# biodatageeks/polars-bio

Measured on AMD Instinct MI355X. Metric: overlap-pairs/sec, higher is better.
Workload: dtype int32; 1 GPU; overlap_100M_5M_24contig; probe_rows=100000000, build_rows=5000000, contigs=24, filter_op=Strict, parallelism=single GPU

## Files before the change

polars-bio_amd/csrc/host_core.hip.h:

```cpp
#pragma once

namespace {

thread_local std::string g_err;

int fail(int code, const std::string& msg) { g_err = msg; return code; }

#define HIP_TRY(expr)                                                                         \
    do {                                                                                      \
        hipError_t _e = (expr);                                                               \
        if (_e != hipSuccess)                                                                 \
            return fail(IVJ_EHIP, std::string(#expr) + ": " + hipGetErrorString(_e));         \
    } while (0)

#define IVJ_ABI_CATCH                                                                                     \
    catch (const std::bad_alloc&) { return fail(IVJ_ENOMEM, "host allocation failed (std::bad_alloc)"); }   \
    catch (const std::exception& e) { return fail(IVJ_ESTATE, std::string("internal error: ") + e.what()); } \
    catch (...) { return fail(IVJ_ESTATE, "internal error: unknown exception"); }

#define IVJ_TRY(expr)                 \
    do {                              \
        int _r = (expr);              \
        if (_r != IVJ_OK) return _r;  \
    } while (0)
// ... 35 lines not shown
        }
    }
};

inline std::atomic<int> g_live_contexts{0};

struct ivj_ctx {
    ivj_ctx() { g_live_contexts.fetch_add(1, std::memory_order_relaxed); }
    ~ivj_ctx() { g_live_contexts.fetch_sub(1, std::memory_order_relaxed); }
    ivj_ctx(const ivj_ctx&) = delete;
    ivj_ctx& operator=(const ivj_ctx&) = delete;
    int device = 0;
    hipStream_t own_stream = nullptr;
    hipStream_t stream = nullptr;
    Arena arena;
    char* ov_buf = nullptr;
    size_t ov_cap = 0;
    int64_t ov_n = -1;
    const void* ov_probe_start = nullptr;
    const void *ov_probe_contig = nullptr, *ov_probe_end = nullptr;
    const ivj_index* ov_ix = nullptr;
    int32_t ov_filter = -1;
    int32_t* ov_hi = nullptr;
    int32_t* ov_cnt = nullptr;
    long long* ov_tile = nullptr;
    long long* h_total = nullptr;
    uint32_t* hw = nullptr;
    uint32_t* hw_dev = nullptr;
    uint32_t hw_seq = 0;
    uint32_t cs_far_hw_seq = 0;
    uint32_t cs_fused_hw_seq = 0;
    int env_spin_us = 4000;
    long long hw_misses = 0;
    bool cs_prep_zero = false;
    XferSlots xfer;
    char* nl_cache = nullptr;
    size_t nl_cache_cap = 0;
    int env_nearest_lines = -1;
    char* ix_cache = nullptr;
    size_t ix_cache_cap = 0;
    int64_t ov_total = 0;
    bool ov_part = false;
    int32_t *pt_c = nullptr, *pt_s = nullptr, *pt_e = nullptr, *pt_row = nullptr;
    uint32_t* pt_off = nullptr; int pt_ntiles = 0;
    uint32_t* pt_bstart = nullptr;
    bool part_attr_set = false;
    bool os_attr_set = false;
    hipEvent_t cs_event = nullptr;
    const ivj_index* cs_far_owner = nullptr;
    hipEvent_t ix3_event = nullptr;
    bool ix3_attr_set = false;
    int env_ix_merge = -1;
    int env_ix_stage = -1;
    int env_ix_v3 = -1;
    int ix3_fallback_streak = 0;
    unsigned ix3_builds_since_fallback = 0;
    int64_t ix3_fallbacks = 0;
    struct StreamBufs { int32_t* h_in = nullptr; int32_t* d_in = nullptr; size_t in_cap = 0; char* d_out = nullptr; size_t d_out_cap = 0;
                        char* h_out = nullptr; size_t h_out_cap = 0; } st_cache[3];
    char* lb_buf = nullptr; size_t lb_cap = 0;
    char* sel_buf = nullptr; size_t sel_cap = 0;
    char* sl_buf = nullptr;
    size_t sl_cap = 0;
    int4* sl_rec = nullptr;
    uint2* sl_cache = nullptr;
    uint32_t *sl_gh = nullptr, *sl_rstart = nullptr, *sl_rcur = nullptr, *sl_bend = nullptr;
    bool sl_sampled = false;
    uint32_t *sl_blk = nullptr, *sl_part = nullptr, *sl_bstart = nullptr;
    int32_t* sl_meta = nullptr;
    int2* sl_map = nullptr;
    long long *sl_tile = nullptr, *sl_tpart = nullptr;
    bool ov_slice = false;
    bool ov_cs = false;
    bool sl_plan_valid = false;
    int sl_items = 2;
    int env_joint_bins = 0, env_count_nolds = 0, env_count_ablate = 0;
    int sl_env_rows = 0, sl_env_chunk = 0, sl_env_notab = 0, sl_env_nobins = 0, sl_env_ablate = 0, sl_env_auto = 1, sl_env_stable = 0, sl_env_sthreads = 1024;
    SlicePlan sl_plan;
    bool cs_sattr_set = false;
    bool cs_attr_set = false;
    int cs_env_walk = -1;
    int cs_env_off = 0;
    int cs_env_ptile = 0;
    int cs_env_fill_two = 0;
    int cs_env_sampled = 1;
    int cs_env_slack = 0;
    int64_t cs_sampled_overflows = 0;
    bool cs_force_exact = false;
    int cs_env_fuse_sample = 1;
    int cs_env_rec8 = 1;
    bool cs_force_rec12 = false;
    int cs_rec8_streak = 0;
    unsigned cs_rec8_skipped = 0;
    bool cs_rec8_tried = false;
    int64_t cs_rec8_overflows = 0;
    int cs_env_nocache = 0;
    int cs_env_persist = 1;
    int cs_env_pmax = 0, cs_env_pgrain = 0;
    int cs_env_pchunks = 0;
    int n_cus = 0;
    const char* cs_env_wgtrace = nullptr;
    unsigned long long* cs_trace_buf = nullptr;
    size_t cs_trace_cap = 0;
    int timing = 0;
    bool t_open = false;
    std::vector<TimingRec> recs;
// ... 284 lines not shown
```

polars-bio_amd/csrc/host_index.hip.h:

```cpp
#pragma once

namespace {

int build_tables(ivj_ctx* ctx, ivj_index* ix);
bool cs_geom(int64_t n, int nc, int want_rows, CsGeom& g);
size_t cs_index_bytes(const CsGeom& g);
void cs_index_carve(ivj_index* ix, char* p);

int ensure_hier(ivj_ctx* ctx, ivj_index* ix) {
    if (ix->hier_built || ix->n <= 0) return IVJ_OK;
    const HierShape h = hier_shape(ix->n);
    const int64_t wgs = (((ix->n + 15) & ~(int64_t)15) + HIER_WG_ROWS - 1) / HIER_WG_ROWS;
    LAUNCH(ctx, "hier_low", k_hier_low, (unsigned)wgs, 256, (const int2*)ix->ep, ix->n, ix->hier, h);
    if (h.nlev >= 3) LAUNCH(ctx, "hier_high", k_hier_high, 1, 256, ix->hier, h, wgs);
    HIP_TRY(hipGetLastError());
    ix->hier_built = true;
    return IVJ_OK;
}

int need_tables(ivj_ctx* ctx, ivj_index* ix) {
    if (!ix->has_tables) return fail(IVJ_ESTATE, "this index was built for merge / cluster only (with_end_order & 2): it has no lookup tables");
    if (ix->tables_built) return IVJ_OK;
    return build_tables(ctx, ix);
}
// ... 176 lines not shown

int build_flat(ivj_ctx* ctx, ivj_index* ix) {
    if (ix->has_flat || ix->n == 0 || ix->n_contigs <= 0) return IVJ_OK;
    IVJ_TRY(need_tables(ctx, ix));
    HIP_TRY(hipMemsetAsync(ix->lot, 0, (size_t)ix->bins_len * 4, ctx->stream));
    LAUNCH(ctx, "lot_mark", k_lot_mark, grid1d(ix->n, 256), 256, (const int2*)ix->ep, (const int32_t*)ix->b_contig, ix->n,
           ix->n_contigs, (const int4*)ix->cmeta, ix->lot);
    IVJ_TRY((lb_scan_u32<MaxOp, false>(ctx, "lot_scan", ix->lot, ix->bins_len, 0u)));
    LAUNCH(ctx, "tab2", k_tab2, grid1d(ix->bins_len, 256), 256, (const uint32_t*)ix->bins, (const uint32_t*)ix->lot, ix->bins_len, ix->tab2);
    HIP_TRY(hipGetLastError());
    IVJ_TRY(build_rec4(ctx, ix));
    ix->has_flat = true;
    return IVJ_OK;
}

int index_sort_v2(ivj_ctx* ctx, ivj_index* ix, const ivj_side* build, const ivj_opts* opts) {
    OsSort S;
    IVJ_TRY(arena_reserve(ctx, os_sort_plan(S, build->n, opts->n_contigs) + 4096));
    os_sort_take(ctx, S);
    IVJ_TRY(os_sort_run(ctx, S, build->contig, build->start, build->end, build->row_id));
    LAUNCH(ctx, "ix_final", k_ix_final, S.tiles, OS_THREADS, (const int4*)S.recA, (const int4*)S.recB, S.n, S.nc, S.cbits, S.meta, S.st_fin, ix->b_start, ix->ep, ix->b_row,
           ix->b_contig, ix->seg, ix->flags);
    HIP_TRY(hipGetLastError());
    return IVJ_OK;
}

bool ix3_wanted(const ivj_ctx* ctx, int64_t n, int nc) {
    if (nc + 1 > V3_MAX_KEYS || n <= 0 || n > (int64_t)V3_CAP * V3_BUCKETS) return false;
    if (ctx->env_ix_v3 >= 0) return ctx->env_ix_v3 != 0;
    if (ctx->ix3_fallback_streak >= 2 && (ctx->ix3_builds_since_fallback & 15) != 15) return false;
    return n >= (128ll << 10) && n <= (7ll << 20);
}
struct V3Plan { int64_t chunk, hist_len, hs_tiles; int nchunks; size_t z_meta, z_st, z_hs, z_tick, zero_bytes; };
V3Plan v3_plan(int64_t n) {
    V3Plan p;
    p.chunk = ((n + 255) / 256 + OS_TILE - 1) / OS_TILE * OS_TILE;
    if (p.chunk < OS_TILE) p.chunk = OS_TILE;
    p.nchunks = (int)((n + p.chunk - 1) / p.chunk);
    p.hist_len = (int64_t)V3_BUCKETS * p.nchunks;
    p.hs_tiles = (p.hist_len + LB_TILE - 1) / LB_TILE;
    p.z_meta = align_up(sizeof(V3Meta)); p.z_st = align_up((size_t)V3_BUCKETS * 8); p.z_hs = align_up((size_t)p.hs_tiles * 8); p.z_tick = align_up(16);
    p.zero_bytes = p.z_meta + p.z_st + p.z_hs + p.z_tick;
    return p;
}
int index_sort_v3(ivj_ctx* ctx, ivj_index* ix, const ivj_side* build, const ivj_opts* opts, bool* done) {
    *done = false;
    const int64_t n = build->n;
    const int nc = opts->n_contigs;
    const int64_t tiles = (n + OS_TILE - 1) / OS_TILE;
    const V3Plan VP = v3_plan(n);
    const int64_t chunk = VP.chunk, hist_len = VP.hist_len, hs_tiles = VP.hs_tiles;
    const int nchunks = VP.nchunks;
    const size_t z_meta = VP.z_meta, z_st = VP.z_st, z_hs = VP.z_hs, zero_bytes = VP.zero_bytes;
    OsSort S;
    const size_t v2_bytes = os_sort_plan(S, n, nc);
    const bool own_z = ix->ix3_z == nullptr;
    IVJ_TRY(arena_reserve(ctx, std::max(v2_bytes, (own_z ? zero_bytes : 0) + align_up((size_t)hist_len * 4) + align_up((size_t)n * 16)) + 4096));
    char* z = own_z ? arena_take<char>(ctx, zero_bytes) : ix->ix3_z;
    uint32_t* hist = arena_take<uint32_t>(ctx, (size_t)hist_len);
    int4* recs = arena_take<int4>(ctx, (size_t)n);
    V3Meta* meta = (V3Meta*)z;
    unsigned long long* st_local = (unsigned long long*)(z + z_meta);
    unsigned long long* st_scan = (unsigned long long*)(z + z_meta + z_st);
    uint32_t* tick_scan = (uint32_t*)(z + z_meta + z_st + z_hs);
    if (own_z) HIP_TRY(hipMemsetAsync(z, 0, zero_bytes, ctx->stream));
    const size_t pass_lds = (size_t)v3_pass_lds().total;
    if (!ctx->ix3_attr_set) {
        HIP_TRY(hipFuncSetAttribute(reinterpret_cast<const void*>(&k_v3_scatter), hipFuncAttributeMaxDynamicSharedMemorySize, (int)pass_lds));
        HIP_TRY(hipFuncSetAttribute(reinterpret_cast<const void*>(&k_v3_local<true>), hipFuncAttributeMaxDynamicSharedMemorySize, 160 * 1024 - 256));
        HIP_TRY(hipFuncSetAttribute(reinterpret_cast<const void*>(&k_v3_local<false>), hipFuncAttributeMaxDynamicSharedMemorySize, 160 * 1024 - 256));
        ctx->ix3_attr_set = true;
    }
    const unsigned sgrid = (unsigned)(tiles < 512 ? tiles : 512);
    LAUNCH(ctx, "ix3_stats", k_v3_stats, sgrid, OS_THREADS, build->start, build->end, build->contig, n, nc, meta);
    LAUNCH(ctx, "ix3_hist", k_v3_hist, nchunks, OS_THREADS, build->contig, build->start, n, nc, meta, (int)chunk, nchunks, hist);
    LAUNCH(ctx, "ix_scan", (k_scan_lb_u32<SumOp, true>), hs_tiles, OS_THREADS, hist, hist_len, 0u, tick_scan, st_scan);
    const int ms_max = ctx->env_ix_merge >= 0 ? std::min(ctx->env_ix_merge, V3_MAX_MERGE) : V3_MAX_MERGE;
    const uint32_t hw_seq = ctx->hw ? ++ctx->hw_seq : 0u;
    LAUNCH(ctx, "ix3_check", k_v3_check, 1, OS_THREADS, (const uint32_t*)hist, nchunks, n, ms_max, meta, ctx->hw_dev, hw_seq);
    if (!ctx->hw) HIP_TRY(hipMemcpyAsync(ctx->h_total + 6, &meta->bad, 8, hipMemcpyDeviceToHost, ctx->stream));
    if (!ctx->ix3_event) HIP_TRY(hipEventCreateWithFlags(&ctx->ix3_event, hipEventDisableTiming));
    HIP_TRY(hipEventRecord(ctx->ix3_event, ctx->stream));
    t_begin(ctx, "ix3_pass");
    hipLaunchKernelGGL(k_v3_scatter, dim3((unsigned)nchunks), dim3(OS_THREADS), pass_lds, ctx->stream, build->contig, build->start, build->end, build->row_id,
                       recs, n, nc, meta, (int)chunk, nchunks, (const uint32_t*)hist);
    t_end(ctx);
    HIP_TRY(hipGetLastError());
    HIP_TRY(wait_event(ctx, ctx->ix3_event));
    uint32_t* hv = reinterpret_cast<uint32_t*>(ctx->h_total + 6);
    if (ctx->hw) {
        const volatile uint32_t* w = reinterpret_cast<volatile uint32_t*>(ctx->hw);
        if (w[2] == hw_seq) { hv[0] = w[0]; hv[1] = w[1]; }
        else {
            ++ctx->hw_misses;
            HIP_TRY(hipMemcpyAsync(ctx->h_total + 6, &meta->bad, 8, hipMemcpyDeviceToHost, ctx->stream));
            HIP_TRY(hipStreamSynchronize(ctx->stream));
        }
    }
    const uint32_t max_bucket = hv[1] & 0xffffffu;
    const int ms = (int)(hv[1] >> 24);
    if (hv[0] != 0u || max_bucket > (uint32_t)V3_CAP) { ++ctx->ix3_fallbacks; ++ctx->ix3_fallback_streak; ctx->ix3_builds_since_fallback = 0; return IVJ_OK; }
    ctx->ix3_fallback_streak = 0;
    const int cap = (int)std::max<uint32_t>(1024u, (max_bucket + 1023u) / 1024u * 1024u);
    const int bin_bits = cap <= 1024 ? 10 : (cap <= 2048 ? 11 : V3_MAX_BIN_BITS);
    const bool stage = ctx->env_ix_stage >= 0 ? ctx->env_ix_stage != 0 : cap <= 2048;
    const size_t local_lds = (size_t)v3_local_lds(cap, 1 << bin_bits, stage).total;
    with_bool(stage, [&](auto STAGE) {
        LAUNCH_LDS(ctx, "ix3_local", k_v3_local<STAGE>, V3_BUCKETS >> ms, OS_THREADS, local_lds, (const int4*)recs, (const uint32_t*)hist, nchunks, n, nc, cap, bin_bits, ms,
                   meta, st_local, ix->b_start, ix->ep, ix->b_row, ix->b_contig, ix->seg, ix->flags);
    });
    HIP_TRY(hipGetLastError());
    *done = true;
    return IVJ_OK;
}

int build_tables(ivj_ctx* ctx, ivj_index* ix) {
    const int nc = ix->n_contigs;
    const int64_t n = ix->n;
    if (n > 0 && nc > 0) {
        const int64_t lb_tiles = (ix->bins_len + LB_TILE - 1) / LB_TILE;
        const size_t zb = align_up((size_t)lb_tiles * 8) + align_up(16);
        IVJ_TRY(arena_reserve(ctx, zb + 4096));
        char* z = arena_take<char>(ctx, zb);
        HIP_TRY(hipMemsetAsync(z, 0, zb, ctx->stream));
        HIP_TRY(hipMemsetAsync(ix->bins, 0, (size_t)ix->bins_len * 4, ctx->stream));
        LAUNCH(ctx, "contig_meta", k_contig_meta, grid1d(nc, 256), 256, (const int32_t*)ix->seg, (const int32_t*)ix->b_start, nc, ix->cmeta);
        LAUNCH(ctx, "bins_mark", k_bins_mark, grid1d(n, 256), 256, (const int32_t*)ix->b_start, (const int32_t*)ix->b_contig, n, nc,
               (const int4*)ix->cmeta, ix->bins);
        LAUNCH(ctx, "bins_scan", (k_scan_lb_u32<MaxOp, false>), lb_tiles, OS_THREADS, ix->bins, ix->bins_len, 0u,
               (uint32_t*)(z + align_up((size_t)lb_tiles * 8)), (unsigned long long*)z);
        LAUNCH(ctx, "bins_records", k_bins_records, grid1d(ix->bins_len, 256), 256, (const uint32_t*)ix->bins, ix->bins_len,
               (const int32_t*)ix->b_start, (const int4*)ix->cmeta, nc, ix->brec);
        HIP_TRY(hipGetLastError());
    }
    ix->tables_built = true;
    return IVJ_OK;
}

int index_build(ivj_ctx* ctx, const ivj_side* build, const ivj_opts* opts, int with_end_order, ivj_index** out) {
    if (2 * build->n + 2 * (int64_t)opts->n_contigs + 64 > 0x7fffffffll)
        return fail(IVJ_EINVAL, "build side too large for the int32 direct-address table (2*rows + 2*contigs must be < 2^31)");
    ivj_index* ix = new ivj_index();
    ix->ctx = ctx; ix->device = ctx->device; ix->n = build->n; ix->n_contigs = opts->n_contigs; ix->table_mode = opts->table_mode;
    const int64_t n = build->n;
    const size_t nn = (size_t)(n > 0 ? n : 1);
    auto cleanup = [&](int code) { ivj_index_free(ix); return code; };
    {
        const size_t col = align_up(nn * 4);
        const size_t nc = (size_t)opts->n_contigs;
        ix->bins_len = 2 * (int64_t)nn + 2 * (int64_t)nc + 16;
        const size_t v3z = (n > 0 && ix3_wanted(ctx, n, opts->n_contigs)) ? v3_plan(n).zero_bytes : 0;
        const size_t small = align_up((nc + 2) * 4) + align_up(16) + 3 * align_up((nc + 1) * 32) + v3z;
        const size_t flat_bytes = align_up((nn + 1) * 16) + 3 * align_up((size_t)ix->bins_len * 4);
        const size_t spl_bytes = align_up((size_t)SL_MAX_BUCKETS * 8) + align_up((size_t)SL_TAB_CONTIGS * 16) +
                                 align_up((size_t)(4 * SL_MAX_BUCKETS + 2 * SL_TAB_CONTIGS) * 4);
        ix->cs_ok = n > 0 && cs_geom(n, opts->n_contigs, opts->slice_rows > 0 ? opts->slice_rows : ctx->sl_env_rows, ix->cs_g);
        const size_t cs_bytes = ix->cs_ok ? cs_index_bytes(ix->cs_g) : 0;
        const size_t hier_bytes = align_up(hier_shape((int64_t)nn).values * 4);
        const size_t need = hier_bytes + cs_bytes + spl_bytes + flat_bytes + 6 * col + align_up(nn * 8) + align_up((nn + 1) * 32) + 2 * align_up((size_t)ix->bins_len * 4) +
                            3 * align_up((size_t)ix->bins_len * 16) + small + 256;
        if (ctx->ix_cache && ctx->ix_cache_cap >= need) {
            ix->slab = ctx->ix_cache; ix->slab_cap = ctx->ix_cache_cap;
// ... 64 lines not shown
```

polars-bio_amd/csrc/ivjoin.hip:

```cpp
#include "../../include/ivjoin.h"

#include <hip/hip_runtime.h>

#include <algorithm>
#include <atomic>
#include <chrono>
#include <cstdio>
#include <cstdlib>
#include <cstring>
#include <string>
#include <vector>
#include <thread>
#include <type_traits>

#include "probe.hip.h"
#include "slice.hip.h"
#include "cslice.hip.h"
#include "onesweep.hip.h"
#include "ixsort3.hip.h"
#include "scan.hip.h"
#include "group.hip.h"
#include "depth.hip.h"
#include "depth_sum.hip.h"
#include "depth_query.hip.h"
// ... 34 lines not shown

int ivj_device_count(int* n) try {
    if (!n) return fail(IVJ_EINVAL, "n is NULL");
    int c = 0;
    hipError_t e = hipGetDeviceCount(&c);
    if (e != hipSuccess) { *n = 0; return fail(IVJ_EHIP, std::string("hipGetDeviceCount: ") + hipGetErrorString(e)); }
    *n = c;
    return IVJ_OK;
} IVJ_ABI_CATCH

int ivj_ctx_create(int device, ivj_ctx** out) try {
    if (!out) return fail(IVJ_EINVAL, "out is NULL");
    int cnt = 0;
    IVJ_TRY(ivj_device_count(&cnt));
    if (device < 0 || device >= cnt) return fail(IVJ_EHIP, "no usable HIP device " + std::to_string(device) + " (device count " + std::to_string(cnt) + ")");
    HIP_TRY(hipSetDevice(device));
    ivj_ctx* ctx = new ivj_ctx();
    ctx->device = device;
    { int cus = 0; if (hipDeviceGetAttribute(&cus, hipDeviceAttributeMultiprocessorCount, device) == hipSuccess) ctx->n_cus = cus; }
    hipError_t e = hipStreamCreateWithFlags(&ctx->own_stream, hipStreamNonBlocking);
    if (e != hipSuccess) { delete ctx; return fail(IVJ_EHIP, std::string("hipStreamCreate: ") + hipGetErrorString(e)); }
    ctx->stream = ctx->own_stream;
    if (const char* ev = std::getenv("IVJ_SLICE_ITEMS")) ctx->sl_items = std::atoi(ev) == 4 ? 4 : 2;
    if (const char* ev = std::getenv("IVJ_SLICE_ROWS")) ctx->sl_env_rows = std::atoi(ev);
    if (const char* ev = std::getenv("IVJ_SLICE_CHUNK")) ctx->sl_env_chunk = std::atoi(ev);
    if (const char* ev = std::getenv("IVJ_SLICE_NOTAB")) ctx->sl_env_notab = std::atoi(ev);
    if (const char* ev = std::getenv("IVJ_SLICE_NOBINS")) ctx->sl_env_nobins = std::atoi(ev);
    if (const char* ev = std::getenv("IVJ_SLICE_ABLATE")) ctx->sl_env_ablate = std::atoi(ev);
    if (const char* ev = std::getenv("IVJ_SLICE_AUTO")) ctx->sl_env_auto = std::atoi(ev);
    if (const char* ev = std::getenv("IVJ_SLICE_STABLE")) ctx->sl_env_stable = std::atoi(ev);
    if (const char* ev = std::getenv("IVJ_SLICE_SCATTER_THREADS")) ctx->sl_env_sthreads = std::atoi(ev);
    if (const char* ev = std::getenv("IVJ_CS")) ctx->cs_env_off = std::atoi(ev) == 0 ? 1 : 0;
    if (const char* ev = std::getenv("IVJ_CS_PTILE")) ctx->cs_env_ptile = std::atoi(ev);
    if (const char* ev = std::getenv("IVJ_CS_NOCACHE")) ctx->cs_env_nocache = std::atoi(ev);
    if (const char* ev = std::getenv("IVJ_CS_PERSIST")) ctx->cs_env_persist = std::atoi(ev);
    if (const char* ev = std::getenv("IVJ_CS_PCHUNKS")) ctx->cs_env_pchunks = std::atoi(ev);
    if (const char* ev = std::getenv("IVJ_CS_PMAX")) ctx->cs_env_pmax = std::atoi(ev);
    if (const char* ev = std::getenv("IVJ_CS_PGRAIN")) ctx->cs_env_pgrain = std::atoi(ev);
    if (const char* ev = std::getenv("IVJ_CS_WGTRACE")) ctx->cs_env_wgtrace = ev[0] ? ev : nullptr;
    if (const char* ev = std::getenv("IVJ_CS_SAMPLED")) ctx->cs_env_sampled = std::atoi(ev);
    if (const char* ev = std::getenv("IVJ_CS_SLACK")) ctx->cs_env_slack = std::atoi(ev);
    if (const char* ev = std::getenv("IVJ_CS_REC8")) ctx->cs_env_rec8 = std::atoi(ev);
    if (const char* ev = std::getenv("IVJ_CS_FUSE_SAMPLE")) ctx->cs_env_fuse_sample = std::atoi(ev);
    if (const char* ev = std::getenv("IVJ_CS_FILL_TWO")) ctx->cs_env_fill_two = std::atoi(ev);
    if (const char* ev = std::getenv("IVJ_CS_WALK")) ctx->cs_env_walk = std::atoi(ev) != 0 ? 1 : 0;
    if (const char* ev = std::getenv("IVJ_JOINT_BINS")) ctx->env_joint_bins = std::atoi(ev);
    if (const char* ev = std::getenv("IVJ_COUNT_ABLATE")) ctx->env_count_ablate = std::atoi(ev);
    if (const char* ev = std::getenv("IVJ_NEAREST_LINES")) ctx->env_nearest_lines = std::atoi(ev);
    if (const char* ev = std::getenv("IVJ_COUNT_NOLDS")) ctx->env_count_nolds = std::atoi(ev);
    if (const char* ev = std::getenv("IVJ_IX_V3")) ctx->env_ix_v3 = std::atoi(ev) != 0 ? 1 : 0;
    if (const char* ev = std::getenv("IVJ_SPIN_US")) ctx->env_spin_us = std::atoi(ev);
    if (const char* ev = std::getenv("IVJ_IX_MERGE")) ctx->env_ix_merge = std::atoi(ev);
    if (const char* ev = std::getenv("IVJ_IX_STAGE")) ctx->env_ix_stage = std::atoi(ev) != 0 ? 1 : 0;
    e = hipHostMalloc((void**)&ctx->h_total, 64, hipHostMallocDefault);
    if (e != hipSuccess) { (void)hipStreamDestroy(ctx->own_stream); delete ctx; return fail(IVJ_EHIP, std::string("hipHostMalloc: ") + hipGetErrorString(e)); }
    {
        const char* ev = std::getenv("IVJ_HOST_WORDS");
        if (!(ev && std::atoi(ev) == 0)) {
            void* hp = nullptr;
            void* dp = nullptr;
            if (hipHostMalloc(&hp, 256, hipHostMallocMapped | hipHostMallocCoherent) == hipSuccess) {
                if (hipHostGetDevicePointer(&dp, hp, 0) == hipSuccess && dp) {
                    std::memset(hp, 0, 256);
                    ctx->hw = (uint32_t*)hp; ctx->hw_dev = (uint32_t*)dp;
                } else (void)hipHostFree(hp);
            }
            (void)hipGetLastError();
        }
    }
    *out = ctx;
    return IVJ_OK;
} IVJ_ABI_CATCH

namespace {
void stream_release(ivj_stream* st, bool keep_cache);
void free_stream_bufs(ivj_ctx::StreamBufs& b) {
    if (b.h_in) (void)hipHostFree(b.h_in);
    if (b.d_in) (void)hipFree(b.d_in);
    if (b.d_out) (void)hipFree(b.d_out);
    if (b.h_out) (void)hipHostFree(b.h_out);
    b = ivj_ctx::StreamBufs();
}
}

void ivj_ctx_destroy(ivj_ctx* ctx) {
    if (!ctx) return;
    DeviceGuard g(ctx->device);
    (void)hipStreamSynchronize(ctx->stream);
    while (!ctx->streams.empty()) stream_release(ctx->streams.back(), false);
    for (ivj_index* ix : ctx->live) ix->ctx = nullptr;
    for (ivj_comm* cm : ctx->comms) comm_detach(cm);
    if (ctx->arena.base) (void)hipFree(ctx->arena.base);
    if (ctx->ov_buf) (void)hipFree(ctx->ov_buf);
    if (ctx->sl_buf) (void)hipFree(ctx->sl_buf);
    if (ctx->cs_trace_buf) (void)hipFree(ctx->cs_trace_buf);
    if (ctx->lb_buf) (void)hipFree(ctx->lb_buf);
    if (ctx->sel_buf) (void)hipFree(ctx->sel_buf);
    for (auto& cb : ctx->st_cache) free_stream_bufs(cb);
    if (ctx->ix_cache) (void)hipFree(ctx->ix_cache);
    if (ctx->nl_cache) (void)hipFree(ctx->nl_cache);
    if (ctx->ix3_event) (void)hipEventDestroy(ctx->ix3_event);
    if (ctx->cs_event) (void)hipEventDestroy(ctx->cs_event);
    if (ctx->h_total) (void)hipHostFree(ctx->h_total);
    if (std::getenv("IVJ_DEBUG_REDO")) std::fprintf(stderr, "[ivj] context: host words %s, %lld misses of %u; ix3 fallbacks %lld\n", ctx->hw ? "on" : "off", (long long)ctx->hw_misses, ctx->hw_seq, (long long)ctx->ix3_fallbacks);
    if (ctx->hw) (void)hipHostFree(ctx->hw);
    ctx->xfer.release();
// ... 1438 lines not shown
```

polars-bio_amd/csrc/ixsort3.hip.h:

```cpp
#pragma once
#include "onesweep.hip.h"

namespace ivj {

constexpr int V3_BUCKETS = OS_RADIX;
constexpr int V3_ITEMS = 4;
constexpr int V3_CAP = OS_THREADS * V3_ITEMS;
constexpr int V3_MAX_KEYS = 256;
constexpr int V3_MAX_BIN_BITS = 12;

struct V3Meta {
    uint32_t inverted;
    uint32_t pad0;
    uint32_t bad;
    uint32_t max_bucket;
    uint32_t ticket;
    uint32_t wbits;
    uint32_t pad[2];
    unsigned long long M;
    unsigned long long span;
    uint32_t cmax[V3_MAX_KEYS];
    uint32_t cimn[V3_MAX_KEYS];
    uint32_t base[V3_MAX_KEYS];
};

__device__ __forceinline__ uint32_t v3_bucket(uint32_t lin, unsigned long long M) { return (uint32_t)(((unsigned long long)lin * M) >> 32); }

__device__ __forceinline__ void v3_load_tables(const V3Meta* __restrict__ meta, int nk, uint32_t* l_base, uint32_t* l_cmin) {
    for (int k = threadIdx.x; k < nk; k += OS_THREADS) { l_base[k] = meta->base[k]; l_cmin[k] = ~meta->cimn[k]; }
}

__global__ __launch_bounds__(OS_THREADS) void k_v3_stats(const int32_t* __restrict__ start, const int32_t* __restrict__ end,
                                                        const int32_t* __restrict__ contig, int64_t n, int32_t n_contigs, V3Meta* __restrict__ meta) {
    __shared__ uint32_t l_mx[V3_MAX_KEYS], l_imn[V3_MAX_KEYS];
    __shared__ uint32_t l_inv;
    const int tid = threadIdx.x, nk = n_contigs + 1;
    for (int k = tid; k < V3_MAX_KEYS; k += OS_THREADS) { l_mx[k] = 0u; l_imn[k] = 0u; }
    if (tid == 0) l_inv = 0u;
    __syncthreads();
    uint32_t inv = 0;
    for (int64_t i = (int64_t)blockIdx.x * OS_THREADS + tid; i < n; i += (int64_t)gridDim.x * OS_THREADS) {
        const int32_t s = start[i], c0 = contig[i];
        const int c = (uint32_t)c0 < (uint32_t)n_contigs ? c0 : n_contigs;
        const uint32_t u = flip(s);
        if (u > l_mx[c]) atomicMax(&l_mx[c], u);
        if (~u > l_imn[c]) atomicMax(&l_imn[c], ~u);
        if (s > end[i] && c < n_contigs) inv = 1u;
    }
    if (inv) l_inv = 1u;
    __syncthreads();
    for (int k = tid; k < nk; k += OS_THREADS) {
        const uint32_t a = l_mx[k], b = l_imn[k];
        if (a > os_ld(&meta->cmax[k])) atomicMax(&meta->cmax[k], a);
        if (b > os_ld(&meta->cimn[k])) atomicMax(&meta->cimn[k], b);
    }
    if (tid == 0 && l_inv && !os_ld(&meta->inverted)) atomicOr(&meta->inverted, 1u);
}

struct V3Geom { unsigned long long M; uint32_t wbits; bool bad; };
__device__ __forceinline__ V3Geom v3_geometry(V3Meta* __restrict__ meta, int nk, uint32_t* l_base, uint32_t* l_cmin, unsigned long long* l_ws , bool record) {
    const int tid = threadIdx.x;
    unsigned long long sp = 0;
// ... 51 lines not shown
                                                        uint32_t* __restrict__ hw, uint32_t hw_seq) {
    __shared__ uint32_t wmx[V3_MAX_MERGE + 1][OS_WAVES];
    if (meta->bad) {
        if (threadIdx.x == 0 && hw) { hw_store(hw + 0, 1u); hw_store(hw + 1, 0u); hw_store(hw + 2, hw_seq); }
        return;
    }
    const int tid = threadIdx.x;
    uint32_t sz[2];
#pragma unroll
    for (int q = 0; q < 2; ++q) {
        const int b = 2 * tid + q;
        const uint32_t a = off[(int64_t)b * nchunks];
        const uint32_t z = b + 1 < V3_BUCKETS ? off[(int64_t)(b + 1) * nchunks] : (uint32_t)n;
        sz[q] = z - a;
    }
    uint32_t mx[V3_MAX_MERGE + 1];
    mx[0] = sz[0] > sz[1] ? sz[0] : sz[1];
    uint32_t sum = sz[0] + sz[1];
    mx[1] = sum;
#pragma unroll
    for (int k = 2; k <= V3_MAX_MERGE; ++k) { sum += __shfl_xor(sum, 1 << (k - 2), kWave); mx[k] = sum; }
#pragma unroll
    for (int k = 0; k <= V3_MAX_MERGE; ++k) {
#pragma unroll
        for (int d = kWave / 2; d > 0; d >>= 1) { const uint32_t o = __shfl_xor(mx[k], d, kWave); mx[k] = o > mx[k] ? o : mx[k]; }
        if ((tid & (kWave - 1)) == 0) wmx[k][tid / kWave] = mx[k];
    }
    __syncthreads();
    if (tid == 0) {
        uint32_t best = 0, best_ms = 0;
#pragma unroll
        for (int k = 0; k <= V3_MAX_MERGE; ++k) {
            uint32_t m = 0;
#pragma unroll
            for (int w = 0; w < OS_WAVES; ++w) m = wmx[k][w] > m ? wmx[k][w] : m;
            if (k == 0 || (k <= ms_max && m <= (uint32_t)V3_CAP)) { best = m; best_ms = (uint32_t)k; }
        }
        meta->max_bucket = best | (best_ms << 24);
        if (hw) { hw_store(hw + 0, 0u); hw_store(hw + 1, best | (best_ms << 24)); hw_store(hw + 2, hw_seq); }
    }
}

struct V3PassLds { OsPassLds P; int tbase, tcmin, total; };
__host__ __device__ inline V3PassLds v3_pass_lds() {
    V3PassLds L;
    L.P = os_pass_lds();
    int o = (L.P.total + 15) & ~15;
    L.tbase = o; o += 4 * V3_MAX_KEYS;
    L.tcmin = o; o += 4 * V3_MAX_KEYS;
    L.total = o;
    return L;
}

__global__ __launch_bounds__(OS_THREADS) void k_v3_scatter(const int32_t* __restrict__ contig, const int32_t* __restrict__ start,
                                                          const int32_t* __restrict__ end, const int32_t* __restrict__ row_id,
                                                          int4* __restrict__ dst, int64_t n, int32_t n_contigs, V3Meta* __restrict__ meta,
                                                          int chunk, int nchunks, const uint32_t* __restrict__ off ) {
    extern __shared__ __attribute__((aligned(16))) unsigned char os_lds[];
    const V3PassLds LL = v3_pass_lds();
    const OsPassLds& L = LL.P;
    int4* l_rec = reinterpret_cast<int4*>(os_lds + L.rec);
    unsigned short* wcnt = reinterpret_cast<unsigned short*>(os_lds + L.wcnt);
    unsigned short* l_d = reinterpret_cast<unsigned short*>(os_lds + L.d);
    uint32_t* base = reinterpret_cast<uint32_t*>(os_lds + L.base);
    uint32_t* lstart = reinterpret_cast<uint32_t*>(os_lds + L.lstart);
    uint32_t* wsum = reinterpret_cast<uint32_t*>(os_lds + L.wsum);
    uint32_t* l_base = reinterpret_cast<uint32_t*>(os_lds + LL.tbase);
    uint32_t* l_cmin = reinterpret_cast<uint32_t*>(os_lds + LL.tcmin);
    if (meta->bad) return;
    const unsigned long long M = meta->M;
    const int tid = threadIdx.x, w = tid / kWave, lane = tid & (kWave - 1);
    v3_load_tables(meta, n_contigs + 1, l_base, l_cmin);
    for (int k = tid; k < OS_RADIX; k += OS_THREADS) base[k] = off[(int64_t)k * nchunks + blockIdx.x];
    for (int k = tid; k < OS_RADIX * OS_WAVES / 2; k += OS_THREADS) reinterpret_cast<uint32_t*>(wcnt)[k] = 0;
    __syncthreads();
    const int64_t cbase = (int64_t)blockIdx.x * chunk;
    const int64_t cend = cbase + chunk < n ? cbase + chunk : n;
    const uint64_t lt = lanemask_lt();
    unsigned short* my = wcnt + w * OS_RADIX;
    const int el0 = w * (OS_ITEMS * kWave) + lane;
    int4 nxt[OS_ITEMS];
    auto load_tile = [&](int64_t tb) {
        const int tn = (int)((cend - tb) < (int64_t)OS_TILE ? (cend - tb) : (int64_t)OS_TILE);
#pragma unroll
        for (int j = 0; j < OS_ITEMS; ++j) {
            const int il = el0 + j * kWave;
            nxt[j] = il < tn ? os_load_record(true, contig, start, end, row_id, nullptr, tb + il, n_contigs) : make_int4(0, 0, 0, 0);
        }
    };
    if (cbase < cend) load_tile(cbase);
    for (int64_t tbase = cbase; tbase < cend; tbase += OS_TILE) {
        const int tile_n = (int)((cend - tbase) < (int64_t)OS_TILE ? (cend - tbase) : (int64_t)OS_TILE);
        int4 r[OS_ITEMS];
        uint32_t d[OS_ITEMS], rank[OS_ITEMS];
#pragma unroll
        for (int j = 0; j < OS_ITEMS; ++j) {
            r[j] = nxt[j];
            d[j] = v3_bucket(l_base[r[j].w] + (flip(r[j].x) - l_cmin[r[j].w]), M);
        }
        if (tbase + OS_TILE < cend) load_tile(tbase + OS_TILE);
#pragma unroll
        for (int j = 0; j < OS_ITEMS; ++j) {
            const bool valid = el0 + j * kWave < tile_n;
            uint64_t peers = __ballot(valid);
#pragma unroll
            for (int b = 0; b < OS_BITS; ++b) {
                const bool bit = (d[j] >> b) & 1u;
                const uint64_t m = __ballot(valid && bit);
                peers &= bit ? m : ~m;
            }
            const uint32_t rk = (uint32_t)__popcll(peers & lt);
            const uint32_t before = valid ? (uint32_t)my[d[j]] : 0u;
            rank[j] = before + rk;
            __builtin_amdgcn_wave_barrier();
            if (valid && rk == 0) my[d[j]] = (unsigned short)(before + (uint32_t)__popcll(peers));
            __builtin_amdgcn_wave_barrier();
        }
        __syncthreads();
        uint32_t x0 = 0, x1 = 0;
        {
            uint32_t* row32 = reinterpret_cast<uint32_t*>(wcnt) + tid;
#pragma unroll
            for (int k = 0; k < OS_WAVES; ++k) {
                const uint32_t v = row32[k * (OS_RADIX / 2)];
                row32[k * (OS_RADIX / 2)] = x0 | (x1 << 16);
                x0 += v & 0xffffu; x1 += v >> 16;
            }
        }
        uint32_t tsum;
        const uint32_t pre = sl_block_exclusive_sum(x0 + x1, wsum, &tsum);
        lstart[2 * tid] = pre;
        lstart[2 * tid + 1] = pre + x0;
        __syncthreads();
#pragma unroll
        for (int j = 0; j < OS_ITEMS; ++j) {
            if (el0 + j * kWave < tile_n) {
                const uint32_t pos = lstart[d[j]] + (uint32_t)my[d[j]] + rank[j];
                l_rec[pos] = r[j];
                l_d[pos] = (unsigned short)d[j];
            }
        }
        __syncthreads();
#pragma unroll
        for (int j = 0; j < OS_ITEMS; ++j) {
            const int il = j * OS_THREADS + tid;
            if (il < tile_n) {
                const uint32_t dd = l_d[il];
                const int4 rr = l_rec[il];
                dst[base[dd] + ((uint32_t)il - lstart[dd])] = rr;
            }
        }
        for (int k = tid; k < OS_RADIX * OS_WAVES / 2; k += OS_THREADS) reinterpret_cast<uint32_t*>(wcnt)[k] = 0;
        __syncthreads();
        base[2 * tid] += x0;
        base[2 * tid + 1] += x1;
        __syncthreads();
    }
}

struct V3LocalLds { int rec, bst, cur, tk, ts, ifin, tbase, tcmin, wsum, total; };
__host__ __device__ inline V3LocalLds v3_local_lds(int cap, int bins, bool stage) {
    V3LocalLds L;
    int o = 0;
    L.rec = o; o += stage ? 16 * cap : 0;
    L.bst = o; o += 4 * (bins + 4);
    L.cur = o; o += 4 * bins;
    L.tk = o; o += 4 * cap;
    L.ts = o; o += 2 * cap;
    L.ifin = o; o += 2 * cap;
    L.tbase = o; o += 4 * V3_MAX_KEYS;
    L.tcmin = o; o += 4 * V3_MAX_KEYS;
    L.wsum = (o + 15) & ~15; o = L.wsum + 8 * OS_WAVES;
    L.total = o;
    return L;
}

template <bool STAGE>
__global__ __launch_bounds__(OS_THREADS, 8) void k_v3_local(const int4* __restrict__ rec, const uint32_t* __restrict__ off, int nchunks, int64_t n,
                                                        int32_t n_contigs, int cap, int bin_bits, int ms, V3Meta* __restrict__ meta, unsigned long long* __restrict__ status64,
                                                        int32_t* __restrict__ b_start, int2* __restrict__ ep, int32_t* __restrict__ b_row,
                                                        int32_t* __restrict__ b_contig, int32_t* __restrict__ seg, int32_t* __restrict__ flags) {
    extern __shared__ __attribute__((aligned(16))) unsigned char os_lds[];
    const int bins = 1 << bin_bits;
    const V3LocalLds L = v3_local_lds(cap, bins, STAGE);
    int4* l_rec = reinterpret_cast<int4*>(os_lds + L.rec);
    uint32_t* bst = reinterpret_cast<uint32_t*>(os_lds + L.bst);
    uint32_t* cur = reinterpret_cast<uint32_t*>(os_lds + L.cur);
    uint32_t* tk = reinterpret_cast<uint32_t*>(os_lds + L.tk);
    unsigned short* ts = reinterpret_cast<unsigned short*>(os_lds + L.ts);
    unsigned short* iF = reinterpret_cast<unsigned short*>(os_lds + L.ifin);
    uint32_t* l_base = reinterpret_cast<uint32_t*>(os_lds + L.tbase);
    uint32_t* l_cmin = reinterpret_cast<uint32_t*>(os_lds + L.tcmin);
    unsigned long long* wmax = reinterpret_cast<unsigned long long*>(os_lds + L.wsum);
    uint32_t* wsum = reinterpret_cast<uint32_t*>(wmax);
    uint32_t* l_pm = tk;
    __shared__ int l_tile;
    __shared__ uint32_t l_lo;
    __shared__ unsigned long long s_carry;
    const int tid = threadIdx.x, w = tid / kWave, lane = tid & (kWave - 1);
    if (tid == 0) {
        const int t = (int)atomicAdd(&meta->ticket, 1u);
        l_tile = t;
        const unsigned long long M = meta->M;
        l_lo = (uint32_t)((((unsigned long long)((unsigned)t << ms) << 32) + M - 1ull) / M);
    }
    v3_load_tables(meta, n_contigs + 1, l_base, l_cmin);
    for (int k = tid; k < bins; k += OS_THREADS) { bst[k] = 0u; cur[k] = 0u; }
    __syncthreads();
    const int tile = l_tile;
    const uint32_t lo = l_lo;
    const int fb0 = tile << ms, fb1 = (tile + 1) << ms;
    const uint32_t b0 = off[(int64_t)fb0 * nchunks];
    const uint32_t b1 = fb1 < V3_BUCKETS ? off[(int64_t)fb1 * nchunks] : (uint32_t)n;
    const int nb = (int)(b1 - b0);
    const int wbits = (int)meta->wbits + ms;
    const int bshift = wbits > bin_bits ? wbits - bin_bits : 0;
    const int4* __restrict__ grec = rec + (int64_t)b0;
    auto row_at = [&](int p) -> int4 { if constexpr (STAGE) return l_rec[p]; else return grec[p]; };

    uint32_t kv[V3_ITEMS];
    unsigned long long cmx = 0ull;
#pragma unroll
    for (int j = 0; j < V3_ITEMS; ++j) {
        const int p = j * OS_THREADS + tid;
        kv[j] = 0u;
        if (p < nb) {
            const int4 r = grec[p];
            if constexpr (STAGE) l_rec[p] = r;
            kv[j] = l_base[r.w] + (flip(r.x) - l_cmin[r.w]) - lo;
            atomicAdd(&bst[kv[j] >> bshift], 1u);
            const unsigned long long c = ((unsigned long long)(uint32_t)r.w << 32) | (unsigned long long)flip(r.y);
            cmx = c > cmx ? c : cmx;
        }
    }
#pragma unroll
    for (int d = kWave / 2; d > 0; d >>= 1) { const unsigned long long o = __shfl_xor(cmx, d, kWave); cmx = o > cmx ? o : cmx; }
    if (lane == 0) wmax[w] = cmx;
    __syncthreads();
    if (tid == 0) {
        unsigned long long tmax = 0;
#pragma unroll
        for (int k = 0; k < OS_WAVES; ++k) tmax = wmax[k] > tmax ? wmax[k] : tmax;
        os_st64(status64 + tile, ((tile == 0 ? 2ull : 1ull) << 62) | tmax);
    }
    {
        const bool own = 4 * tid < bins;
        uint4 c4 = make_uint4(0u, 0u, 0u, 0u);
        if (own) c4 = *reinterpret_cast<const uint4*>(bst + 4 * tid);
        const uint32_t s = c4.x + c4.y + c4.z + c4.w;
        __syncthreads();
        uint32_t tsum;
        uint32_t pre = sl_block_exclusive_sum<uint32_t>(s, wsum, &tsum);
        uint4 o4;
        o4.x = pre; pre += c4.x; o4.y = pre; pre += c4.y; o4.z = pre; pre += c4.z; o4.w = pre;
        if (own) *reinterpret_cast<uint4*>(bst + 4 * tid) = o4;
        if (tid == 0) bst[bins] = (uint32_t)nb;
    }
    __syncthreads();
#pragma unroll
    for (int j = 0; j < V3_ITEMS; ++j) {
        const int p = j * OS_THREADS + tid;
        if (p < nb) {
            const uint32_t bin = kv[j] >> bshift;
            const uint32_t q = bst[bin] + atomicAdd(&cur[bin], 1u);
            tk[q] = kv[j];
            ts[q] = (unsigned short)p;
        }
    }
    __syncthreads();
#pragma unroll
    for (int j = 0; j < V3_ITEMS; ++j) {
        const int p = j * OS_THREADS + tid;
        if (p < nb) {
            const uint32_t bin = kv[j] >> bshift;
            const uint32_t a = bst[bin], z = bst[bin + 1];
            uint32_t r = a;
            for (uint32_t q = a; q < z; ++q) {
                const uint32_t k2 = tk[q];
                const uint32_t s2 = ts[q];
                r += (k2 < kv[j] || (k2 == kv[j] && s2 < (uint32_t)p)) ? 1u : 0u;
// ... 32 lines not shown
        const unsigned long long VAL = (1ull << 62) - 1ull;
        unsigned long long carry = 0;
        for (int t0 = tile - 1; t0 >= 0; t0 -= kWave) {
            const int t = t0 - lane;
            unsigned long long v = 2ull << 62;
            if (t >= 0) {
                v = os_ld64(status64 + t);
                while ((v >> 62) == 0) { __builtin_amdgcn_s_sleep(2); v = os_ld64(status64 + t); }
            }
            const unsigned long long pre_mask = __ballot((v >> 62) == 2ull);
            const int first = pre_mask ? __builtin_ctzll(pre_mask) : kWave;
            unsigned long long x = lane <= first ? (v & VAL) : 0ull;
#pragma unroll
            for (int d = kWave / 2; d > 0; d >>= 1) { const unsigned long long o = __shfl_xor(x, d, kWave); x = o > x ? o : x; }
            carry = x > carry ? x : carry;
            if (pre_mask) break;
        }
        if (lane == 0) s_carry = carry;
    }
    __syncthreads();
    unsigned long long wpre = 0, tmax = 0;
#pragma unroll
    for (int k = 0; k < OS_WAVES; ++k) { const unsigned long long x = wmax[k]; if (k < w) wpre = x > wpre ? x : wpre; tmax = x > tmax ? x : tmax; }
    unsigned long long excl = __shfl_up(inc, 1, kWave);
    if (lane == 0) excl = 0;
    excl = wpre > excl ? wpre : excl;
    if (tid == 0) {
        if (tile > 0) os_st64(status64 + tile, (2ull << 62) | (s_carry > tmax ? s_carry : tmax));
        if (tile == 0) flags[0] = (int32_t)meta->inverted;
    }
    const unsigned long long before = s_carry > excl ? s_carry : excl;
    if (tid == 0) prev_c = b0 == 0u ? -1 : (int32_t)(s_carry >> 32);
#pragma unroll
    for (int k = 0; k < V3_ITEMS; ++k) {
        const int q = V3_ITEMS * tid + k;
        if (q < nb) {
            const unsigned long long pm = before > comp[k] ? before : comp[k];
            l_pm[q] = (uint32_t)pm;
            const int64_t p = (int64_t)b0 + q;
            for (int32_t kk = prev_c + 1; kk <= cc[k]; ++kk) seg[kk] = (int32_t)p;
            prev_c = cc[k];
            if (p == n - 1) for (int32_t kk = cc[k] + 1; kk <= n_contigs + 1; ++kk) seg[kk] = (int32_t)n;
        }
    }
    __syncthreads();
#pragma unroll
    for (int j = 0; j < V3_ITEMS; ++j) {
        const int q = j * OS_THREADS + tid;
        if (q < nb) {
            const int4 r = row_at(iF[q]);
            const int64_t g = (int64_t)b0 + q;
            b_start[g] = r.x;
            ep[g] = make_int2(r.y, unflip(l_pm[q]));
            b_row[g] = r.z;
            b_contig[g] = r.w;
        }
    }
}

}
```

Measured before the change: 112.3 billion overlap-pairs/s.

## Pack index-sort records into 12 bytes with row position and contig bits

Adds a 12-byte record format for the v3 index sort. The row position (23 bits) and the contig key (9 bits) are packed into one word, so intermediate records shrink from 16 to 12 bytes in global memory and LDS during scatter. The final row id is gathered from the original row_id array in the local-sort pass. This is on by default and cuts scatter write bandwidth and record reads, at the cost of an extra indirect gather and non-16B-aligned accesses. It only affects index build time within the join.

```diff
diff --git a/polars-bio_amd/csrc/host_core.hip.h b/polars-bio_amd/csrc/host_core.hip.h
--- a/polars-bio_amd/csrc/host_core.hip.h
+++ b/polars-bio_amd/csrc/host_core.hip.h
@@ -111,6 +111,7 @@
     bool ix3_attr_set = false;
     int env_ix_merge = -1;
     int env_ix_stage = -1;
+    int env_ix_rec12 = -1;
     int env_ix_v3 = -1;
     int ix3_fallback_streak = 0;
     unsigned ix3_builds_since_fallback = 0;
diff --git a/polars-bio_amd/csrc/host_index.hip.h b/polars-bio_amd/csrc/host_index.hip.h
--- a/polars-bio_amd/csrc/host_index.hip.h
+++ b/polars-bio_amd/csrc/host_index.hip.h
@@ -252,13 +252,15 @@
     const int64_t chunk = VP.chunk, hist_len = VP.hist_len, hs_tiles = VP.hs_tiles;
     const int nchunks = VP.nchunks;
     const size_t z_meta = VP.z_meta, z_st = VP.z_st, z_hs = VP.z_hs, zero_bytes = VP.zero_bytes;
+    const bool rec12 = ctx->env_ix_rec12 != 0;
+    const size_t rec_bytes = rec12 ? sizeof(V3Rec12) : sizeof(int4);
     OsSort S;
     const size_t v2_bytes = os_sort_plan(S, n, nc);
     const bool own_z = ix->ix3_z == nullptr;
-    IVJ_TRY(arena_reserve(ctx, std::max(v2_bytes, (own_z ? zero_bytes : 0) + align_up((size_t)hist_len * 4) + align_up((size_t)n * 16)) + 4096));
+    IVJ_TRY(arena_reserve(ctx, std::max(v2_bytes, (own_z ? zero_bytes : 0) + align_up((size_t)hist_len * 4) + align_up((size_t)n * rec_bytes)) + 4096));
     char* z = own_z ? arena_take<char>(ctx, zero_bytes) : ix->ix3_z;
     uint32_t* hist = arena_take<uint32_t>(ctx, (size_t)hist_len);
-    int4* recs = arena_take<int4>(ctx, (size_t)n);
+    int4* recs = arena_take<int4>(ctx, ((size_t)n * rec_bytes + 15) / 16);
     V3Meta* meta = (V3Meta*)z;
     unsigned long long* st_local = (unsigned long long*)(z + z_meta);
     unsigned long long* st_scan = (unsigned long long*)(z + z_meta + z_st);
@@ -266,9 +268,12 @@
     if (own_z) HIP_TRY(hipMemsetAsync(z, 0, zero_bytes, ctx->stream));
     const size_t pass_lds = (size_t)v3_pass_lds().total;
     if (!ctx->ix3_attr_set) {
-        HIP_TRY(hipFuncSetAttribute(reinterpret_cast<const void*>(&k_v3_scatter), hipFuncAttributeMaxDynamicSharedMemorySize, (int)pass_lds));
-        HIP_TRY(hipFuncSetAttribute(reinterpret_cast<const void*>(&k_v3_local<true>), hipFuncAttributeMaxDynamicSharedMemorySize, 160 * 1024 - 256));
-        HIP_TRY(hipFuncSetAttribute(reinterpret_cast<const void*>(&k_v3_local<false>), hipFuncAttributeMaxDynamicSharedMemorySize, 160 * 1024 - 256));
+        IVJ_TRY(with_bool(rec12, [&](auto R) {
+            HIP_TRY(hipFuncSetAttribute(reinterpret_cast<const void*>(&k_v3_scatter<R>), hipFuncAttributeMaxDynamicSharedMemorySize, (int)pass_lds));
+            HIP_TRY(hipFuncSetAttribute(reinterpret_cast<const void*>(&k_v3_local<true, R>), hipFuncAttributeMaxDynamicSharedMemorySize, 160 * 1024 - 256));
+            HIP_TRY(hipFuncSetAttribute(reinterpret_cast<const void*>(&k_v3_local<false, R>), hipFuncAttributeMaxDynamicSharedMemorySize, 160 * 1024 - 256));
+            return (int)IVJ_OK;
+        }));
         ctx->ix3_attr_set = true;
     }
     const unsigned sgrid = (unsigned)(tiles < 512 ? tiles : 512);
@@ -282,8 +287,10 @@
     if (!ctx->ix3_event) HIP_TRY(hipEventCreateWithFlags(&ctx->ix3_event, hipEventDisableTiming));
     HIP_TRY(hipEventRecord(ctx->ix3_event, ctx->stream));
     t_begin(ctx, "ix3_pass");
-    hipLaunchKernelGGL(k_v3_scatter, dim3((unsigned)nchunks), dim3(OS_THREADS), pass_lds, ctx->stream, build->contig, build->start, build->end, build->row_id,
-                       recs, n, nc, meta, (int)chunk, nchunks, (const uint32_t*)hist);
+    with_bool(rec12, [&](auto R) {
+        hipLaunchKernelGGL(k_v3_scatter<R>, dim3((unsigned)nchunks), dim3(OS_THREADS), pass_lds, ctx->stream, build->contig, build->start, build->end, build->row_id,
+                           (void*)recs, n, nc, meta, (int)chunk, nchunks, (const uint32_t*)hist);
+    });
     t_end(ctx);
     HIP_TRY(hipGetLastError());
     HIP_TRY(wait_event(ctx, ctx->ix3_event));
@@ -305,9 +312,9 @@
     const int bin_bits = cap <= 1024 ? 10 : (cap <= 2048 ? 11 : V3_MAX_BIN_BITS);
     const bool stage = ctx->env_ix_stage >= 0 ? ctx->env_ix_stage != 0 : cap <= 2048;
     const size_t local_lds = (size_t)v3_local_lds(cap, 1 << bin_bits, stage).total;
-    with_bool(stage, [&](auto STAGE) {
-        LAUNCH_LDS(ctx, "ix3_local", k_v3_local<STAGE>, V3_BUCKETS >> ms, OS_THREADS, local_lds, (const int4*)recs, (const uint32_t*)hist, nchunks, n, nc, cap, bin_bits, ms,
-                   meta, st_local, ix->b_start, ix->ep, ix->b_row, ix->b_contig, ix->seg, ix->flags);
+    with_bool(stage, rec12, [&](auto STAGE, auto R) {
+        LAUNCH_LDS(ctx, "ix3_local", (k_v3_local<STAGE, R>), V3_BUCKETS >> ms, OS_THREADS, local_lds, (const void*)recs, (const int32_t*)build->row_id, (const uint32_t*)hist,
+                   nchunks, n, nc, cap, bin_bits, ms, meta, st_local, ix->b_start, ix->ep, ix->b_row, ix->b_contig, ix->seg, ix->flags);
     });
     HIP_TRY(hipGetLastError());
     *done = true;
diff --git a/polars-bio_amd/csrc/ivjoin.hip b/polars-bio_amd/csrc/ivjoin.hip
--- a/polars-bio_amd/csrc/ivjoin.hip
+++ b/polars-bio_amd/csrc/ivjoin.hip
@@ -110,6 +110,7 @@
     if (const char* ev = std::getenv("IVJ_SPIN_US")) ctx->env_spin_us = std::atoi(ev);
     if (const char* ev = std::getenv("IVJ_IX_MERGE")) ctx->env_ix_merge = std::atoi(ev);
     if (const char* ev = std::getenv("IVJ_IX_STAGE")) ctx->env_ix_stage = std::atoi(ev) != 0 ? 1 : 0;
+    if (const char* ev = std::getenv("IVJ_IX_REC12")) ctx->env_ix_rec12 = std::atoi(ev) != 0 ? 1 : 0;
     e = hipHostMalloc((void**)&ctx->h_total, 64, hipHostMallocDefault);
     if (e != hipSuccess) { (void)hipStreamDestroy(ctx->own_stream); delete ctx; return fail(IVJ_EHIP, std::string("hipHostMalloc: ") + hipGetErrorString(e)); }
     {
diff --git a/polars-bio_amd/csrc/ixsort3.hip.h b/polars-bio_amd/csrc/ixsort3.hip.h
--- a/polars-bio_amd/csrc/ixsort3.hip.h
+++ b/polars-bio_amd/csrc/ixsort3.hip.h
@@ -8,6 +8,12 @@
 constexpr int V3_CAP = OS_THREADS * V3_ITEMS;
 constexpr int V3_MAX_KEYS = 256;
 constexpr int V3_MAX_BIN_BITS = 12;
+
+constexpr int V3_POS_BITS = 23;
+constexpr uint32_t V3_POS_MASK = (1u << V3_POS_BITS) - 1u;
+static_assert((int64_t)V3_CAP * V3_BUCKETS <= (1ll << V3_POS_BITS) && (7ll << 20) <= (1ll << V3_POS_BITS), "a row position of the balanced build fits 23 bits");
+static_assert(V3_MAX_KEYS <= 512, "a contig key fits the 9 bits above the row position");
+struct __attribute__((aligned(4))) V3Rec12 { int32_t x, y; uint32_t z; };
 
 struct V3Meta {
     uint32_t inverted;
@@ -165,14 +171,18 @@
     return L;
 }
 
+template <bool REC12>
 __global__ __launch_bounds__(OS_THREADS) void k_v3_scatter(const int32_t* __restrict__ contig, const int32_t* __restrict__ start,
                                                           const int32_t* __restrict__ end, const int32_t* __restrict__ row_id,
-                                                          int4* __restrict__ dst, int64_t n, int32_t n_contigs, V3Meta* __restrict__ meta,
+                                                          void* __restrict__ dst_, int64_t n, int32_t n_contigs, V3Meta* __restrict__ meta,
                                                           int chunk, int nchunks, const uint32_t* __restrict__ off ) {
     extern __shared__ __attribute__((aligned(16))) unsigned char os_lds[];
     const V3PassLds LL = v3_pass_lds();
     const OsPassLds& L = LL.P;
     int4* l_rec = reinterpret_cast<int4*>(os_lds + L.rec);
+    uint32_t* l_rec32 = reinterpret_cast<uint32_t*>(os_lds + L.rec);
+    int4* __restrict__ dst = reinterpret_cast<int4*>(dst_);
+    V3Rec12* __restrict__ dst12 = reinterpret_cast<V3Rec12*>(dst_);
     unsigned short* wcnt = reinterpret_cast<unsigned short*>(os_lds + L.wcnt);
     unsigned short* l_d = reinterpret_cast<unsigned short*>(os_lds + L.d);
     uint32_t* base = reinterpret_cast<uint32_t*>(os_lds + L.base);
@@ -198,7 +208,7 @@
 #pragma unroll
         for (int j = 0; j < OS_ITEMS; ++j) {
             const int il = el0 + j * kWave;
-            nxt[j] = il < tn ? os_load_record(true, contig, start, end, row_id, nullptr, tb + il, n_contigs) : make_int4(0, 0, 0, 0);
+            nxt[j] = il < tn ? os_load_record(true, contig, start, end, REC12 ? nullptr : row_id, nullptr, tb + il, n_contigs) : make_int4(0, 0, 0, 0);
         }
     };
     if (cbase < cend) load_tile(cbase);
@@ -249,7 +259,12 @@
         for (int j = 0; j < OS_ITEMS; ++j) {
             if (el0 + j * kWave < tile_n) {
                 const uint32_t pos = lstart[d[j]] + (uint32_t)my[d[j]] + rank[j];
-                l_rec[pos] = r[j];
+                if constexpr (REC12) {
+                    l_rec32[3 * pos] = (uint32_t)r[j].x; l_rec32[3 * pos + 1] = (uint32_t)r[j].y;
+                    l_rec32[3 * pos + 2] = (uint32_t)r[j].z | ((uint32_t)r[j].w << V3_POS_BITS);
+                } else {
+                    l_rec[pos] = r[j];
+                }
                 l_d[pos] = (unsigned short)d[j];
             }
         }
@@ -259,8 +274,14 @@
             const int il = j * OS_THREADS + tid;
             if (il < tile_n) {
                 const uint32_t dd = l_d[il];
-                const int4 rr = l_rec[il];
-                dst[base[dd] + ((uint32_t)il - lstart[dd])] = rr;
+                if constexpr (REC12) {
+                    V3Rec12 rr;
+                    rr.x = (int32_t)l_rec32[3 * il]; rr.y = (int32_t)l_rec32[3 * il + 1]; rr.z = l_rec32[3 * il + 2];
+                    dst12[base[dd] + ((uint32_t)il - lstart[dd])] = rr;
+                } else {
+                    const int4 rr = l_rec[il];
+                    dst[base[dd] + ((uint32_t)il - lstart[dd])] = rr;
+                }
             }
         }
         for (int k = tid; k < OS_RADIX * OS_WAVES / 2; k += OS_THREADS) reinterpret_cast<uint32_t*>(wcnt)[k] = 0;
@@ -288,8 +309,8 @@
     return L;
 }
 
-template <bool STAGE>
-__global__ __launch_bounds__(OS_THREADS, 8) void k_v3_local(const int4* __restrict__ rec, const uint32_t* __restrict__ off, int nchunks, int64_t n,
+template <bool STAGE, bool REC12>
+__global__ __launch_bounds__(OS_THREADS, 8) void k_v3_local(const void* __restrict__ rec, const int32_t* __restrict__ row_id, const uint32_t* __restrict__ off, int nchunks, int64_t n,
                                                         int32_t n_contigs, int cap, int bin_bits, int ms, V3Meta* __restrict__ meta, unsigned long long* __restrict__ status64,
                                                         int32_t* __restrict__ b_start, int2* __restrict__ ep, int32_t* __restrict__ b_row,
                                                         int32_t* __restrict__ b_contig, int32_t* __restrict__ seg, int32_t* __restrict__ flags) {
@@ -328,8 +349,13 @@
     const int nb = (int)(b1 - b0);
     const int wbits = (int)meta->wbits + ms;
     const int bshift = wbits > bin_bits ? wbits - bin_bits : 0;
-    const int4* __restrict__ grec = rec + (int64_t)b0;
-    auto row_at = [&](int p) -> int4 { if constexpr (STAGE) return l_rec[p]; else return grec[p]; };
+    const int4* __restrict__ grec = reinterpret_cast<const int4*>(rec) + (int64_t)b0;
+    const V3Rec12* __restrict__ grec12 = reinterpret_cast<const V3Rec12*>(rec) + (int64_t)b0;
+    auto load_g = [&](int p) -> int4 {
+        if constexpr (REC12) { const V3Rec12 t = grec12[p]; return make_int4(t.x, t.y, (int32_t)(t.z & V3_POS_MASK), (int32_t)(t.z >> V3_POS_BITS)); }
+        else return grec[p];
+    };
+    auto row_at = [&](int p) -> int4 { if constexpr (STAGE) return l_rec[p]; else return load_g(p); };
 
     uint32_t kv[V3_ITEMS];
     unsigned long long cmx = 0ull;
@@ -338,7 +364,7 @@
         const int p = j * OS_THREADS + tid;
         kv[j] = 0u;
         if (p < nb) {
-            const int4 r = grec[p];
+            const int4 r = load_g(p);
             if constexpr (STAGE) l_rec[p] = r;
             kv[j] = l_base[r.w] + (flip(r.x) - l_cmin[r.w]) - lo;
             atomicAdd(&bst[kv[j] >> bshift], 1u);
@@ -477,7 +503,8 @@
             const int64_t g = (int64_t)b0 + q;
             b_start[g] = r.x;
             ep[g] = make_int2(r.y, unflip(l_pm[q]));
-            b_row[g] = r.z;
+            if constexpr (REC12) b_row[g] = row_id ? row_id[r.z] : r.z;
+            else b_row[g] = r.z;
             b_contig[g] = r.w;
         }
     }
```

Measured after the change: 112.5 billion overlap-pairs/s, median of 4. No clear change (+0.2%).
